# anneouyang/OuterSPACE

Hardware: AMD Instinct MI355X
Metric: spgemm_output_nnz_per_s (higher is better)
Workload: dtype f64

## Files before the change

outerspace_amd/csrc/osp_kernels.h:

```cpp
#pragma once
#include <type_traits>
#include "osp_prims.h"

namespace osp {

template <class T> struct TileCap;
#ifndef OSP_TILE_CAP_F32
#define OSP_TILE_CAP_F32 1792
#endif
template <> struct TileCap<float> { static constexpr int value = OSP_TILE_CAP_F32; };
#ifndef OSP_TILE_CAP_F64
#define OSP_TILE_CAP_F64 1536
#endif
template <> struct TileCap<double> { static constexpr int value = OSP_TILE_CAP_F64; };
constexpr int kMergeThreads = 256;
constexpr int kTileMaxRows = kMergeThreads - 1;
constexpr int kMulThreads = 256;
#ifndef OSP_MUL_PER_WAVE
#define OSP_MUL_PER_WAVE 2048
#endif
constexpr int kMulPerWave = OSP_MUL_PER_WAVE;
constexpr int kMulPerBlock = kMulPerWave * (kMulThreads / kWave);
#ifndef OSP_MUL_BATCH_MAX
#define OSP_MUL_BATCH_MAX 4096
#endif
constexpr int kMulBatchMax = OSP_MUL_BATCH_MAX;
constexpr int kMulBatchAvg = 64;
#ifndef OSP_MUL_TILE_MIN
#define OSP_MUL_TILE_MIN 1024
#endif
#ifndef OSP_MUL_QU_MID
#define OSP_MUL_QU_MID 2
#endif
#ifndef OSP_MUL_QU_HUB
#define OSP_MUL_QU_HUB 1
#endif
constexpr int kMulTileMin = OSP_MUL_TILE_MIN;
constexpr int kMulTileW = 128;

template <class T>
struct __attribute__((packed, aligned(4))) Part {
    uint32_t col;
    T val;
};

template <class T>
struct __attribute__((packed, aligned(4))) PartWords {
    uint32_t w[sizeof(Part<T>) / 4];
    __device__ __forceinline__ uint32_t col() const { return w[0]; }
    __device__ __forceinline__ T val() const {
        if constexpr (sizeof(T) == 8) return (T)__hiloint2double((int)w[2], (int)w[1]);
        else return (T)__uint_as_float(w[1]);
    }
};
template <class T>
__device__ __forceinline__ PartWords<T> load_part_words(const Part<T> *p) { return *reinterpret_cast<const PartWords<T> *>(p); }
template <class T>
__device__ __forceinline__ void store_part_words(Part<T> *p, const PartWords<T> &r) { *reinterpret_cast<PartWords<T> *>(p) = r; }

#ifndef OSP_NT_STAGE
#define OSP_NT_STAGE 1
#endif
template <class T>
__device__ __forceinline__ void stream_store_part(Part<T> *p, uint32_t col, T val) {
#if OSP_NT_STAGE
    if constexpr (sizeof(T) == 8) {
        typedef uint32_t u32x3 __attribute__((ext_vector_type(3), aligned(4)));
        const uint64_t b = (uint64_t)__double_as_longlong((double)val);
        u32x3 v;
        v.x = col; v.y = (uint32_t)b; v.z = (uint32_t)(b >> 32);
        __builtin_nontemporal_store(v, reinterpret_cast<u32x3 *>(p));
    } else {
        typedef uint32_t u32x2 __attribute__((ext_vector_type(2), aligned(4)));
        u32x2 v;
        v.x = col; v.y = __float_as_uint((float)val);
        __builtin_nontemporal_store(v, reinterpret_cast<u32x2 *>(p));
    }
#else
    *p = Part<T>{col, val};
#endif
}

constexpr uint32_t kFlagRange = 1u, kFlagUnsorted = 2u, kFlagDuplicate = 4u, kFlagPtr = 8u;

template <class T, class X>
__device__ __forceinline__ uint64_t upper_bound_dev(const T *a, uint64_t lo, uint64_t hi, X x) {
    while (lo < hi) {
        uint64_t mid = (lo + hi) >> 1;
        if ((X)a[mid] <= x) lo = mid + 1; else hi = mid;
    }
    return lo;
}
template <class T, class X>
__device__ __forceinline__ uint64_t wave_upper_bound(const T *a, uint64_t lo, uint64_t hi, X x) {
    const uint64_t lane = lane_id();
    while (hi - lo > 64) {
        const uint64_t step = (hi - lo) / 64, p = lo + lane * step;
        const int c = __popcll(__ballot((X)a[p] <= x));
        if (c == 0) return lo;
        if (c < 64) hi = lo + (uint64_t)c * step;
        lo = lo + (uint64_t)(c - 1) * step + 1;
    }
    const bool le = lane < hi - lo && (X)a[lo + lane] <= x;
    return lo + (uint64_t)__popcll(__ballot(le));
}
template <class T, class X>
__device__ __forceinline__ uint64_t lower_bound_dev(const T *a, uint64_t lo, uint64_t hi, X x) {
    while (lo < hi) {
        uint64_t mid = (lo + hi) >> 1;
        if ((X)a[mid] < x) lo = mid + 1; else hi = mid;
    }
    return lo;
// ... 439 lines not shown
                            const bool there = q + i < cj;
                            const uint32_t qi = there ? q + i : q;
                            const uint64_t j = jb + qi;
                            av[i] = wave_bcast(av_l, qi);
                            off[i] = there ? wave_bcast(off_l, qi) : kChunkSkip;
                            ok[i] = in && off[i] != kChunkSkip && !(j == j0 && l < la) && !(j == j1 && l >= lb);
                        }
                        bool dir[QU];
                        chunk_dests<T, QU, MODE>(cells, hub, ri, chunk_off, stage, qstage, off, l, l, bc, dst, dir);
#pragma unroll
                        for (int i = 0; i < QU; i++)
                            if (ok[i]) store_dest<T, MODE>(dst[i], off[i], dir[i], bc, av[i] * bv);
                    }
                }
            }
        } else {
            const uint32_t g = kWave / nb;
            const uint32_t jj = (lane * ((65536u + nb - 1) / nb)) >> 16;
            const uint32_t l = lane - jj * nb;
            const bool in = jj < g;
            uint32_t bc = 0; T bv = 0;
            if (in) { bc = b_colidx[bs + l]; bv = b_vals[bs + l]; }
            for (uint64_t jb = j0; jb <= j1; jb += g) {
                const uint64_t j = jb + jj;
                bool ok = in && j <= j1 && !(j == j0 && l < la) && !(j == j1 && l >= lb);
                if (ok) {
                    uint64_t e = as + j;
                    if constexpr (IND) e = elist[e];
                    const uint64_t raw = chunk_off[e - (uint64_t)e0];
                    if (raw != kChunkSkip) {
                        if (DIRECT && (raw & kDirectBit)) store_direct<T, MODE>(cells, hub, qstage, raw, bs, l, bc, a_vals[e] * bv);
                        else stream_store_part(&stage[raw - base + l], bc, a_vals[e] * bv);
                    }
                }
            }
        }
        cur = p0 + b;
    }
    if constexpr (!IND) return;
    }
}

constexpr int kExpandThreads = 256;
constexpr uint32_t kExpandJob = 8192;
struct ExpandJobs {
    const uint32_t *rows; const uint64_t *row_off; const uint8_t *hmode; uint8_t mode_a, mode_b;
    __device__ uint64_t operator()(uint64_t h) const {
        const uint8_t m = hmode[h];
        if (m != mode_a && m != mode_b) return 0ull;
        const uint64_t U = row_off[rows[h] + 1] - row_off[rows[h]];
        return (U + kExpandJob - 1) / kExpandJob;
    }
};
template <class T>
__global__ __launch_bounds__(kExpandThreads) void expand_rows_kernel(
    const uint32_t *__restrict__ rows, uint32_t nlong, const uint64_t *__restrict__ jobbase, const uint64_t *__restrict__ row_off, uint64_t base,
    const uint32_t *__restrict__ rowfirst, const uint64_t *__restrict__ ct_off, const uint32_t *__restrict__ ct_bs, const uint32_t *__restrict__ perm,
    const T *__restrict__ a_vals, const uint32_t *__restrict__ b_colidx, const T *__restrict__ b_vals, Part<T> *__restrict__ stage) {
    const uint64_t job = blockIdx.x;
    if (job >= jobbase[nlong]) return;
    const unsigned lane = lane_id(), w = threadIdx.x >> 6;
    const uint32_t h = (uint32_t)(upper_bound_dev(jobbase, 0, (uint64_t)nlong + 1, job) - 1);
    const uint32_t row = rows[h];
    const uint64_t rbeg = row_off[row], rend = row_off[row + 1];
    constexpr uint32_t per = kExpandJob / (kExpandThreads / kWave);
    const uint64_t p0 = rbeg + (job - jobbase[h]) * kExpandJob + (uint64_t)w * per;
    if (p0 >= rend) return;
    const uint64_t p1 = min(p0 + per, rend);
    const uint32_t c0 = rowfirst[row], c1 = rowfirst[row + 1];
    uint32_t c = (uint32_t)(upper_bound_dev(ct_off, (uint64_t)c0, (uint64_t)c1, p0) - 1);
    constexpr uint32_t kUnroll = 4;
    for (; c < c1; c += kWave) {
        const uint32_t cq = c + lane;
        const bool cv = cq < c1;
        const uint64_t o0 = cv ? ct_off[cq] : ~0ull, o1 = cv ? ct_off[cq + 1] : ~0ull;
        if (wave_bcast(o0, 0u) >= p1) break;
        const uint32_t bsv = cv ? ct_bs[cq] : 0u;
        const T av = cv ? (perm ? a_vals[perm[cq]] : a_vals[cq]) : T(0);
        const uint64_t g0 = max(wave_bcast(o0, 0u), p0);
        const uint32_t nval = min((uint32_t)kWave, c1 - c);
        const uint64_t g1 = min(wave_bcast(o1, nval - 1), p1);
        for (uint64_t ib = g0; ib < g1; ib += kUnroll * kWave) {
            uint32_t bc[kUnroll];
            T bv[kUnroll], cav[kUnroll];
#pragma unroll
            for (uint32_t u = 0; u < kUnroll; u++) {
                const uint64_t i = ib + u * kWave + lane;
                uint32_t lo = 0, hi = kWave;
#pragma unroll
                for (int step = 0; step < 6; step++) {
                    const uint32_t mid = (lo + hi) >> 1;
                    const uint64_t sv = (uint64_t)__shfl((long long)o0, (int)mid);
                    if (sv <= i) lo = mid; else hi = mid;
                }
                const uint64_t cst = (uint64_t)__shfl((long long)o0, (int)lo);
                const uint32_t cbs = (uint32_t)__shfl((int)bsv, (int)lo);
                cav[u] = __shfl(av, (int)lo);
                const uint32_t b = i < g1 ? cbs + (uint32_t)(i - cst) : 0u;
                bc[u] = b_colidx[b];
                bv[u] = b_vals[b];
            }
#pragma unroll
            for (uint32_t u = 0; u < kUnroll; u++) {
                const uint64_t i = ib + u * kWave + lane;
                if (i < g1) stream_store_part(&stage[i - base], bc[u], cav[u] * bv[u]);
            }
        }
    }
}

struct CoarseStartFlag {
    const uint64_t *row_off;
    uint64_t r0, base, slot;
    const uint8_t *force;
    __device__ uint32_t operator()(uint64_t t) const {
        if (t == 0) return 1;
        const uint64_t r = r0 + t;
        if (force && force[t]) return 1;
        return ((row_off[r] - base) / slot != (row_off[r - 1] - base) / slot || (t & 0xffffu) == 0) ? 1u : 0u;
    }
};
__global__ void tile_walk_kernel(const uint32_t *cb_rows, const uint32_t *ncb_p, uint32_t ncb_max, uint64_t r_end, const uint64_t *row_off,
                                 uint64_t cap, uint32_t max_rows, const uint32_t *tile_base, uint32_t *counts,
                                 uint32_t *tile_rows) {
    const uint32_t j = blockIdx.x * blockDim.x + threadIdx.x;
    const uint32_t ncb = *ncb_p;
    if (j >= ncb) {
        if (!tile_rows && j < ncb_max) counts[j] = 0;
        return;
    }
    uint64_t r = cb_rows[j];
    const uint64_t end = (j + 1 < ncb) ? (uint64_t)cb_rows[j + 1] : r_end;
    uint32_t n = 0;
    const uint32_t out = tile_rows ? tile_base[j] : 0u;
    while (r < end) {
        if (tile_rows) tile_rows[out + n] = (uint32_t)r;
        const uint64_t lim = min(end, r + max_rows);
        uint64_t r2 = upper_bound_dev(row_off, r + 1, lim + 1, row_off[r] + cap) - 1;
        if (r2 <= r) r2 = r + 1;
        r = r2;
        n++;
    }
    if (!tile_rows) counts[j] = n;
}
struct HeavyRowFlag {
    const uint64_t *row_off;
    uint64_t r0;
    uint32_t kTileCap;
    __device__ uint32_t operator()(uint64_t t) const {
        const uint64_t r = r0 + t;
        return (row_off[r + 1] - row_off[r]) > (uint64_t)kTileCap ? 1u : 0u;
    }
};
template <class F>
__global__ void compact_flagged_kernel(F f, const uint32_t *scan, uint64_t n, uint64_t r0,
                                       uint32_t *list) {
    uint64_t t = (uint64_t)blockIdx.x * blockDim.x + threadIdx.x;
    if (t < n && f(t)) list[scan[t]] = (uint32_t)(r0 + t);
}

constexpr uint64_t kStatusAgg = 1ull << 62, kStatusPrefix = 2ull << 62, kStatusMask = (1ull << 62) - 1;
// ... 1364 lines not shown
```

outerspace_amd/csrc/osp_pipeline.h:

```cpp
#pragma once

#define OSP_WITH_RA(ctx_, ...)                                               \
    do {                                                                     \
        if ((ctx_)->rank_atomic) { constexpr bool RA = true; __VA_ARGS__; }  \
        else { constexpr bool RA = false; __VA_ARGS__; }                     \
    } while (0)

template <class T> struct Producer {
    virtual ~Producer() {}
    virtual void produce(uint64_t r0, uint64_t r1, bool whole, uint64_t base, uint64_t count,
                         Part<T> *stage, PhaseTimer &tm, const uint32_t *cells = nullptr, Part<T> *qstage = nullptr,
                         const HubArgs *hub = nullptr, bool compact = false, bool has_long = true, bool desc_only = false, bool walk_all = false) = 0;
};

template <class T> struct MergeIO {
    Part<T> *stage;
    const uint64_t *row_off; uint64_t r0, r1, base;
    int64_t *c_rowptr; uint32_t *c_col; T *c_val;
    const uint64_t *out_in; uint64_t *out_out;
    ChunkTable<T> ct{};
    uint32_t *abort_word = nullptr;
    const RunDesc<T> *runs0 = nullptr; const uint32_t *rowfirst0 = nullptr; const uint32_t *b_colidx = nullptr; const T *b_vals = nullptr;
};
template <class T> struct ShortRuns {
// ... 34 lines not shown
    pl.tile_rows = sc.get<uint32_t>((uint64_t)pl.ntiles + 1);
    tile_walk_kernel<<<grid_for(ncb, 128), 128, 0, s>>>(tmp_rows, ncb_p, ncb, r1, row_off, cap, max_rows, cb_cnt, nullptr, pl.tile_rows);
    return pl;
}

struct DirectSrc {
    const uint32_t *rowfirst; const uint64_t *off; const uint32_t *bs; const uint32_t *perm; const uint32_t *b_colidx;
    uint64_t *chunk_off;
    uint64_t direct_max;
    const int64_t *b_rowptr = nullptr;
    uint64_t K = 0, nnz_b = 0;
    Scratch *keep = nullptr;
    mutable HubTables hub{};
    mutable bool hub_refused = false;
    bool gather = false;
    bool expand_rows = false;
    mutable bool chunk_off_ready = true;
    const uint32_t *rows_sorted = nullptr;
    const uint64_t *row_off = nullptr;
    uint64_t rw_cap = 0, nnz = 0;
    void ensure_chunk_off(hipStream_t s) const {
        if (chunk_off_ready) return;
        sym_scatter_offsets_kernel<<<grid_for(nnz, 256), 256, 0, s>>>(perm, off, rows_sorted, row_off, rw_cap, nnz, chunk_off);
        chunk_off_ready = true;
    }
    const void *a_vals = nullptr, *b_vals = nullptr;
    bool av_in_order = false;
    unsigned long long *gstat = nullptr;
};

template <class T> struct PanelPlan {
    Scratch sc;
    TilePlan p0;
    uint32_t max_rows = 0;
    uint64_t *hoff = nullptr, *hscan_tmp = nullptr, *blkbase = nullptr, *hbase = nullptr, *vbase = nullptr, *cellbase = nullptr;
    uint8_t *hbits = nullptr, *hmode = nullptr;
    uint32_t *nstretch = nullptr;
    uint64_t nh = 0, nblocks = 0, nvirt = 0, ncell = 0;
    uint64_t mode_rows[3] = {0, 0, 0}, mode_partials[3] = {0, 0, 0};
    uint32_t *ghist = nullptr, *ghist_tmp = nullptr;
    Part<T> *qstage = nullptr;
    uint64_t *vrow_off = nullptr;
    uint8_t *vfirst = nullptr;
    uint32_t *vcol0 = nullptr, *vcol1 = nullptr;
    uint32_t *cells = nullptr;
    HubArgs hub{};
    GatherArgs<T> ga{};
    uint32_t *vrun_off = nullptr, *vrun_end = nullptr;
    uint32_t *nwritten = nullptr;
    uint64_t *xjobbase = nullptr;
    uint64_t xjobs_bound = 0, xpartials = 0;
    bool expand_ok = false;
    bool may_write = false;
    explicit PanelPlan(Context *c) : sc(c) {}
};

__global__ void mode_totals_kernel(const uint32_t *rows, uint32_t nlong, const uint64_t *row_off, const uint8_t *hmode,
                                   const uint8_t *hsmall, unsigned long long *totals) {
    uint64_t part[3] = {0, 0, 0}, cnt[3] = {0, 0, 0}, nsmall = 0;
    for (uint32_t h = blockIdx.x * blockDim.x + threadIdx.x; h < nlong; h += gridDim.x * blockDim.x) {
        const uint64_t U = row_off[rows[h] + 1] - row_off[rows[h]];
        const uint8_t m = hmode[h];
        nsmall += hsmall[h] ? 1ull : 0ull;
#pragma unroll
        for (int mode = 0; mode < 3; mode++) { part[mode] += m == mode ? U : 0ull; cnt[mode] += m == mode ? 1ull : 0ull; }
    }
    for (uint8_t mode = 0; mode < 3; mode++) {
        const uint64_t p = wave_reduce_sum<uint64_t>(part[mode]), c = wave_reduce_sum<uint64_t>(cnt[mode]);
        if (lane_id() == 0 && c) { atomicAdd(&totals[mode], (unsigned long long)c); atomicAdd(&totals[3 + mode], (unsigned long long)p); }
    }
    nsmall = wave_reduce_sum<uint64_t>(nsmall);
    if (lane_id() == 0 && nsmall) atomicAdd(&totals[6], (unsigned long long)nsmall);
}

template <class T>
static void plan_panel(Context *ctx, Result *res, PhaseTimer &tm, PanelPlan<T> &pl, const uint64_t *row_off, uint64_t r0, uint64_t r1,
                       uint64_t base, uint64_t count, int colbits, const DirectSrc *ds) {
    hipStream_t s = ctx->stream;
    Scratch &sc = pl.sc;
    constexpr uint32_t kCap = (uint32_t)TileCap<T>::value;
    pl.max_rows = (uint32_t)std::min<uint64_t>(kTileMaxRows, colbits >= 32 ? 1ull : (1ull << (32 - colbits)));
    pl.p0 = plan_tiles(ctx, sc, row_off, r0, r1, base, kCap, pl.max_rows, nullptr, count, 0);
    res->info.light_tiles += pl.p0.ntiles - pl.p0.nlong;
    if (!pl.p0.nlong) return;
    const uint32_t nlong = pl.p0.nlong;
    pl.hoff = sc.get<uint64_t>((uint64_t)nlong + 1);
    pl.hscan_tmp = sc.get<uint64_t>(scan_scratch_entries(nlong));
    device_exclusive_scan<HeavyLen, uint64_t>(HeavyLen{pl.p0.long_rows, row_off}, nlong, pl.hoff, pl.hscan_tmp, s);
    pl.hbits = sc.get<uint8_t>(nlong);
    pl.hmode = sc.get<uint8_t>(nlong);
    pl.nstretch = sc.get<uint32_t>(nlong);
    uint32_t *nseg = sc.get<uint32_t>(nlong);
    uint64_t *nhist = sc.get<uint64_t>(nlong), *ncellh = sc.get<uint64_t>(nlong);
    const bool want_gather = ds && ds->gather;
    uint64_t *nrund = want_gather ? sc.get<uint64_t>(nlong) : nullptr, *rdbase = want_gather ? sc.get<uint64_t>((uint64_t)nlong + 1) : nullptr;
    uint64_t nrd = 0;
    pl.blkbase = sc.get<uint64_t>((uint64_t)nlong + 1); pl.hbase = sc.get<uint64_t>((uint64_t)nlong + 1);
    pl.vbase = sc.get<uint64_t>((uint64_t)nlong + 1); pl.cellbase = sc.get<uint64_t>((uint64_t)nlong + 1);
    unsigned long long *totals = (unsigned long long *)sc.get<uint64_t>(7);
    uint8_t *hsmall = sc.get<uint8_t>(nlong);
    SmallLimits small_lim{};
    if (want_gather && !(getenv("OSP_PLAN_SMALL") && atoi(getenv("OSP_PLAN_SMALL")) == 0) &&
        !(getenv("OSP_GATHER_OVER") && atoi(getenv("OSP_GATHER_OVER")) == 0)) {
        small_lim.cells = (uint32_t)std::clamp<long>(getenv("OSP_PLAN_SMALL_CELLS") ? atol(getenv("OSP_PLAN_SMALL_CELLS")) : (long)kSmallCells,
                                                     (long)kSmallCellsMin, (long)kSmallCellsMax);
        small_lim.chunks = (uint32_t)std::clamp<long>(getenv("OSP_PLAN_SMALL_CHUNKS") ? atol(getenv("OSP_PLAN_SMALL_CHUNKS")) : (long)kSmallChunks,
// ... 140 lines not shown
            uint32_t *scan_tmp = tmp.get<uint32_t>(scan_scratch_entries(nb + 1));
            OSP_HIP(hipMemsetAsync(rowstart, 0, nb + 4, s));
            hub_rowstart_kernel<<<grid_for(ds->K, 256), 256, 0, s>>>(ds->b_rowptr, ds->K, rowstart);
            const int sh = colbits - hub_b;
            const HubRunFlag flag{rowstart, ds->b_colidx, sh};
            device_exclusive_scan<HubRunFlag, uint32_t>(flag, nb, sx, scan_tmp, s);
            compact_flagged_kernel<HubRunFlag><<<grid_for(nb, 256), 256, 0, s>>>(flag, sx, nb, 0, runstart);
            hub_runstart_end_kernel<<<1, 1, 0, s>>>(sx + nb, runstart, (uint32_t)nb);
            OSP_HIP(hipMemsetAsync(runblk, 0, (nb + 2) * sizeof(uint16_t), s));
            hub_runblk_kernel<<<std::min(grid_for(nb, 256), 4096u), 256, 0, s>>>(sx + nb, runstart, ds->b_colidx, sh, runblk);
            OSP_HIP(hipStreamSynchronize(s));
            ds->hub.sx = sx; ds->hub.runstart = runstart; ds->hub.runblk = runblk; ds->hub.sh = sh;
        }
        tm.begin(PH_HUB_K, s);
        uint64_t *jobruns = sc.get<uint64_t>(pl.nblocks + 1);
        uint64_t *jobscan_tmp = sc.get<uint64_t>(scan_scratch_entries(pl.nblocks + 1));
        const size_t hub_lds = sizeof(uint32_t) << hub_b;
        hub_plan_kernel<false><<<(unsigned)pl.nblocks, kHubThreads, hub_lds, s>>>(pl.p0.long_rows, nlong, pl.blkbase, pl.hbase, pl.hbits, pl.nstretch, row_off,
                                                                           ds->rowfirst, ds->off, ds->bs, ds->perm, ds->b_colidx, ds->hub, pl.ghist,
                                                                           pl.hoff, jobruns, nullptr, nullptr, nullptr);
        device_exclusive_scan<LoadU32, uint32_t>(LoadU32{pl.ghist}, pl.ncell, pl.ghist, pl.ghist_tmp, s);
        device_exclusive_scan<LoadU64, uint64_t>(LoadU64{jobruns}, pl.nblocks, jobruns, jobscan_tmp, s);
        const uint64_t ncells = d2h(jobruns + pl.nblocks, s);
        if (ncells >= (1ull << 40)) throw Error(OSP_ERR_CAPACITY, "hub rows: too many runs in one panel");
        if (getenv("OSP_VERBOSE"))
            fprintf(stderr, "[osp]   hub rows: %llu rows, %llu products in %llu runs (%.2f records per run), %llu jobs, 2^%d blocks\n",
                    (unsigned long long)pl.mode_rows[kModeStretch], (unsigned long long)pl.mode_partials[kModeStretch], (unsigned long long)ncells,
                    ncells ? (double)pl.mode_partials[kModeStretch] / (double)ncells : 0.0, (unsigned long long)pl.nblocks, hub_b);
        const double min_run = getenv("OSP_HUB_MIN_RUN") ? atof(getenv("OSP_HUB_MIN_RUN")) : 4.0;
        const double run = ncells ? (double)pl.mode_partials[kModeStretch] / (double)ncells : 0.0;
        const bool accept = run >= min_run;
        if (!accept) {
            ds->hub_refused = true;
            tm.end(PH_HUB_K);
        } else {
            uint32_t *hcells = sc.get<uint32_t>(ncells);
            ds->ensure_chunk_off(s);
            hub_plan_kernel<true><<<(unsigned)pl.nblocks, kHubThreads, hub_lds, s>>>(pl.p0.long_rows, nlong, pl.blkbase, pl.hbase, pl.hbits, pl.nstretch, row_off,
                                                                              ds->rowfirst, ds->off, ds->bs, ds->perm, ds->b_colidx, ds->hub, pl.ghist,
                                                                              pl.hoff, nullptr, jobruns, hcells, ds->chunk_off);
            tm.end(PH_HUB_K);
            pl.hub.cells = hcells;
            pl.hub.sx = ds->hub.sx;
            res->info.hub_plan_launches++;
            res->info.hub_cells += ncells;
            res->info.hub_rows += pl.mode_rows[kModeStretch];
            res->info.hub_partials += pl.mode_partials[kModeStretch];
        }
        dbg_sync(s, "plan of the hub rows");
    }
    if (ds && ds->expand_rows) {
        pl.expand_ok = true;
        const bool hubs = pl.hub.cells != nullptr;
        const uint64_t rows_x = pl.mode_rows[kModeSplitRow] + (hubs ? 0 : pl.mode_rows[kModeStretch]);
        pl.xpartials = pl.mode_partials[kModeSplitRow] + (hubs ? 0 : pl.mode_partials[kModeStretch]);
        if (rows_x) {
            pl.xjobbase = sc.get<uint64_t>((uint64_t)nlong + 1);
            device_exclusive_scan<ExpandJobs, uint64_t>(ExpandJobs{pl.p0.long_rows, row_off, pl.hmode, kModeSplitRow, hubs ? kModeSplitRow : kModeStretch},
                                                        nlong, pl.xjobbase, pl.hscan_tmp, s);
            pl.xjobs_bound = pl.xpartials / kExpandJob + rows_x;
        }
    }
}

template <class T>
static void merge_panel(Context *ctx, Result *res, PhaseTimer &tm, const MergeIO<T> &io, int colbits, PanelPlan<T> &pl) {
    hipStream_t s = ctx->stream;
    Scratch &sc = pl.sc;
    constexpr uint32_t kCap = (uint32_t)TileCap<T>::value;
    const uint32_t max_rows = pl.max_rows;
#ifdef OSP_CHECK_DESC
    crumbs_init();
#endif
    const uint64_t r1 = io.r1, base = io.base;
    const TilePlan &p0 = pl.p0;

    MergeLevels<T> lv{};
    lv.stage[0] = io.stage; lv.row_off[0] = io.row_off; lv.base[0] = base; lv.c_rowptr[0] = io.c_rowptr; lv.heavy_nnz[0] = nullptr;
    uint32_t ntot = p0.ntiles;
    TileDesc *desc = nullptr;
    TilePlan p1;
    uint64_t *vbase = pl.vbase;
    int64_t *vptr = nullptr;
    uint64_t *seg_src = nullptr;
    uint32_t *seg_nnz = nullptr;
    Part<T> *qstage = pl.qstage;
    if (p0.nlong) {
        const uint32_t nlong = p0.nlong;
        uint64_t *hoff = pl.hoff, *hscan_tmp = pl.hscan_tmp, *blkbase = pl.blkbase, *hbase = pl.hbase;
        uint8_t *hbits = pl.hbits;
        uint32_t *nstretch = pl.nstretch, *ghist = pl.ghist, *ghist_tmp = pl.ghist_tmp;
        const uint64_t nh = pl.nh, nblocks = pl.nblocks, nvirt = pl.nvirt, ncell = pl.ncell;
        uint64_t *vrow_off = pl.vrow_off;
        uint8_t *vfirst = pl.vfirst;
        if (pl.mode_rows[kModeSplitRow]) {
            tm.begin(PH_SPLIT_K);
            OSP_WITH_RA(ctx, split_row_kernel<T, RA><<<nlong, kSplitRowThreads, 0, s>>>(p0.long_rows, nlong, hbits, pl.hmode, vbase, hoff, io.row_off,
                                                                                     base, colbits, io.stage, qstage, vrow_off));
            tm.end(PH_SPLIT_K);
            res->info.split_launches++;
            res->info.split_partials += pl.mode_partials[kModeSplitRow];
            dbg_sync(s, "split: one-workgroup rows");
        }
        if (nblocks && !pl.hub.cells) {
            split_count_kernel<<<(unsigned)nblocks, kSplitThreads, 0, s>>>(p0.long_rows, nlong, blkbase, hbase, hbits, nstretch, io.row_off,
                                                                         base, colbits, (const char *)io.stage, (uint32_t)sizeof(Part<T>), ghist);
            device_exclusive_scan<LoadU32, uint32_t>(LoadU32{ghist}, ncell, ghist, ghist_tmp, s);
            OSP_WITH_RA(ctx, split_scatter_kernel<T, RA><<<(unsigned)nblocks, kSplitThreads, 0, s>>>(
                                 p0.long_rows, nlong, blkbase, hbase, hbits, nstretch, io.row_off, base, colbits, io.stage, ghist, hoff, qstage));
        }
        dbg_sync(s, "split: stretch rows");
        split_vrows_kernel<<<grid_for(nvirt + 1, 256), 256, 0, s>>>(nlong, vbase, hbase, nstretch, hbits, pl.hmode, colbits, ghist, hoff, nvirt, nh,
                                                                   vrow_off, vfirst, pl.vcol0, pl.vcol1);
        OSP_HIP(hipGetLastError());
        dbg_sync(s, "split: segment offsets");
        p1 = plan_tiles(ctx, sc, vrow_off, 0, nvirt, 0, kCap, max_rows, vfirst, nh, nlong);
        dbg_sync(s, "tiles over the segments");
        vptr = (int64_t *)sc.get<uint64_t>(nvirt + 1);
        lv.stage[1] = qstage; lv.row_off[1] = vrow_off; lv.base[1] = 0; lv.c_rowptr[1] = vptr;
        if (p1.nlong) {
            const uint32_t nseg_long = p1.nlong;
            seg_src = sc.get<uint64_t>(nseg_long);
            seg_nnz = sc.get<uint32_t>(nvirt + 1);
            lv.heavy_nnz[1] = seg_nnz;
            if (pl.ga.runs) {
                uint64_t *xsjob = sc.get<uint64_t>((uint64_t)nseg_long + 1);
                uint64_t *xsjob_tmp = sc.get<uint64_t>(scan_scratch_entries((uint64_t)nseg_long + 1));
                device_exclusive_scan<SegExpandJobs, uint64_t>(SegExpandJobs{p1.long_rows, vrow_off, pl.vrun_off}, nseg_long, xsjob, xsjob_tmp, s);
                const uint64_t job_bound = nh / kExpandJob + nseg_long;
                expand_segments_kernel<T><<<(unsigned)std::min<uint64_t>(job_bound, (uint64_t)ctx->cus * 8), kExpandThreads, 0, s>>>(
                    p1.long_rows, nseg_long, xsjob, vrow_off, pl.vrun_off, pl.vrun_end, pl.ga.runs, pl.ga.b_colidx, pl.ga.b_vals, qstage);
            }
            const uint32_t *rest_list = p1.long_rows;
            uint32_t nrest = nseg_long;
            uint32_t *hscan = sc.get<uint32_t>((uint64_t)nseg_long + 1);
            uint64_t *sscan_tmp = sc.get<uint64_t>(scan_scratch_entries(nseg_long));
            {
                const SegDenseFlag df{p1.long_rows, pl.vcol0, pl.vcol1, getenv("OSP_DENSE_SEG") ? atoi(getenv("OSP_DENSE_SEG")) : 1};
                device_exclusive_scan<SegDenseFlag, uint32_t>(df, nseg_long, hscan, (uint32_t *)sscan_tmp, s);
                const uint32_t ndense = d2h(hscan + nseg_long, s);
                if (ndense) {
                    uint32_t *dense_list = sc.get<uint32_t>(ndense), *others = sc.get<uint32_t>(nseg_long - ndense);
                    seg_split_list_kernel<SegDenseFlag><<<grid_for(nseg_long, 256), 256, 0, s>>>(df, hscan, nseg_long, dense_list, others);
                    if (ctx->dense_atomic[sizeof(T) == 8])
                        dense_segment_kernel<T, true><<<grid_for(ndense, kDenseWaves), kDenseWaves * kWave, 0, s>>>(dense_list, ndense, vrow_off, pl.vcol0, pl.vcol1,
                                                                              qstage, seg_nnz);
                    else
                        dense_segment_kernel<T, false><<<grid_for(ndense, kDenseWaves), kDenseWaves * kWave, 0, s>>>(dense_list, ndense, vrow_off, pl.vcol0, pl.vcol1,
                                                                              qstage, seg_nnz);
                    res->info.dense_segments += ndense;
                    rest_list = others;
                    nrest = nseg_long - ndense;
                }
            }
            dbg_sync(s, "over-long segments: dense accumulation");
            const uint32_t big_cap = getenv("OSP_BIGTILE_CAP") ? std::min<uint32_t>((uint32_t)strtoul(getenv("OSP_BIGTILE_CAP"), nullptr, 10), kBigTileCap)
                                                                : (uint32_t)kBigTileCap;
            uint32_t nhuge = 0, nmid = 0;
            uint32_t *huge_list = nullptr, *mid_list = nullptr;
            if (nrest) {
                const SegHugeFlag hf{rest_list, vrow_off, big_cap};
                device_exclusive_scan<SegHugeFlag, uint32_t>(hf, nrest, hscan, (uint32_t *)sscan_tmp, s);
                nhuge = d2h(hscan + nrest, s);
                nmid = nrest - nhuge;
                huge_list = sc.get<uint32_t>(nhuge);
                mid_list = sc.get<uint32_t>(nmid);
// ... 244 lines not shown
    for (uint32_t p = 0; p < npanels; p++) {
        max_panel = std::max(max_panel, panel_count(p));
        max_rows_panel = std::max(max_rows_panel, bounds[p + 1] - bounds[p]);
    }
    Part<T> *stage = sc.get<Part<T>>(max_panel);
    uint64_t *out_nnz = sc.get<uint64_t>((uint64_t)npanels + 1);
    uint32_t *abort_word = sc.get<uint32_t>(1);
    zero_async(s, {{out_nnz, sizeof(uint64_t)}, {abort_word, sizeof(uint32_t)}});
    auto check_abort = [&](uint32_t flag) {
        if (flag) throw Error(OSP_ERR_HIP, "the merge made no progress for seconds (a tile's predecessors never published their sizes); "
                                           "with several ticket shards that happens when fewer workgroups than shards ever run side by side");
    };
    const bool overlap = npanels > 1 && !(getenv("OSP_PLAN_OVERLAP") && atoi(getenv("OSP_PLAN_OVERLAP")) == 0);
    if (overlap) ctx->need_aux();
    struct AuxScope {
        Context *c; hipStream_t main;
        explicit AuxScope(Context *ctx_) : c(ctx_), main(ctx_->stream) { c->stream = c->aux; }
        ~AuxScope() {
            if (std::uncaught_exceptions()) (void)hipStreamSynchronize(c->aux);
            c->stream = main;
        }
    };
    typedef std::unique_ptr<PanelPlan<T>> PlanPtr;
    auto plan_one = [&](uint32_t p, bool beside) -> PlanPtr {
        const uint64_t r0 = bounds[p], r1 = bounds[p + 1];
        const uint64_t base = panel_base(p), count = panel_count(p);
        PlanPtr pl(new PanelPlan<T>(ctx));
        if (beside) {
            AuxScope scope(ctx);
            OSP_HIP(hipStreamWaitEvent(ctx->stream, ctx->aux_fork, 0));
            tm.begin(PH_MERGE, ctx->stream);
            plan_panel<T>(ctx, res, tm, *pl, d_row_off, r0, r1, base, count, colbits, ds);
            tm.end(PH_MERGE);
            OSP_HIP(hipEventRecord(ctx->aux_join, ctx->stream));
            res->info.plans_overlapped++;
        } else {
            tm.begin(PH_MERGE);
            plan_panel<T>(ctx, res, tm, *pl, d_row_off, r0, r1, base, count, colbits, ds);
            tm.end(PH_MERGE);
        }
        return pl;
    };
    auto multiply_and_plan_next = [&](uint32_t p, PanelPlan<T> &plan, PlanPtr &nxt) {
        const uint64_t r0 = bounds[p], r1 = bounds[p + 1];
        const uint64_t base = panel_base(p), count = panel_count(p);
        if (plan.p0.nlong) plan.qstage = plan.sc.template get<Part<T>>(plan.nh);
        const bool beside = overlap && p + 1 < npanels;
        if (beside) { OSP_HIP(hipEventRecord(ctx->aux_fork, s)); ctx->fork_window = true; ctx->releases_in_fork_window = 0; }
        struct WindowEnd { Context *c; ~WindowEnd() { c->fork_window = false; } } window_end{ctx};
        tm.begin(PH_MUL);
        bool column_major = count != 0 && !(sr && plan.p0.nlong == 0), desc_only = false;
        if (count && plan.xjobbase && plan.xjobs_bound) {
            tm.begin(PH_EXPAND_K);
            expand_rows_kernel<T><<<(unsigned)plan.xjobs_bound, kExpandThreads, 0, s>>>(plan.p0.long_rows, plan.p0.nlong, plan.xjobbase, d_row_off, base, ds->rowfirst,
                                                                                     ds->off, ds->bs, ds->av_in_order ? nullptr : ds->perm, (const T *)ds->a_vals,
                                                                                     ds->b_colidx, (const T *)ds->b_vals, stage);
            tm.end(PH_EXPAND_K);
            res->info.expand_launches++;
            res->info.expand_partials += plan.xpartials;
        }
        if (count && plan.expand_ok) {
            desc_only = true;
            const uint32_t nw = (plan.nwritten && plan.may_write) ? d2h(plan.nwritten, s) : 0u;
            column_major = plan.hub.cells != nullptr || nw != 0 || (plan.mode_rows[kModeDirect] != 0 && plan.ga.runs == nullptr);
        }
        const bool mostly_hub = plan.hub.cells != nullptr && plan.mode_partials[kModeStretch] * 3 >= count;
        if (column_major && ds) ds->ensure_chunk_off(s);
        if (column_major) prod.produce(r0, r1, npanels == 1 && all_rows, base, count, stage, tm, plan.cells, plan.qstage, plan.hub.cells ? &plan.hub : nullptr,
                                       plan.ga.runs != nullptr && !mostly_hub, plan.p0.nlong != 0, desc_only, mostly_hub);
        tm.end(PH_MUL);
        if (beside) {
            ctx->fork_window = false;
            if (ctx->releases_in_fork_window)
                throw Error(OSP_ERR_HIP, "internal: " + std::to_string(ctx->releases_in_fork_window) + " pooled buffers were released between the fork of the "
                                         "second stream and the next panel's plan (the pool is not stream-aware: see Context::fork_window)");
            nxt = plan_one(p + 1, true);
            OSP_HIP(hipStreamWaitEvent(s, ctx->aux_join, 0));
        }
    };
    if (sink) {
        std::vector<uint64_t> h_ub(npanels + 1);
        for (uint32_t p = 0; p <= npanels; p++) h_ub[p] = d2h(ub + (bounds[p] - r_lo), s);
        uint64_t max_out = 1;
        for (uint32_t p = 0; p < npanels; p++) max_out = std::max(max_out, h_ub[p + 1] - h_ub[p]);
        c_col = sc.get<uint32_t>(max_out);
        c_val = sc.get<T>(max_out);
        int64_t *prow = sc.get<int64_t>(max_rows_panel + 1);
        uint64_t *cells = sc.get<uint64_t>(2);
        uint64_t nnz_total = 0;
        PlanPtr cur, nxt;
        for (uint32_t p = 0; p < npanels; p++) {
            const uint64_t r0 = bounds[p], r1 = bounds[p + 1];
            const uint64_t base = panel_base(p);
            if (!cur) cur = plan_one(p, false);
            PanelPlan<T> &plan = *cur;
            multiply_and_plan_next(p, plan, nxt);
            tm.begin(PH_MERGE);
            OSP_HIP(hipMemsetAsync(cells, 0, 2 * sizeof(uint64_t), s));
            MergeIO<T> io{stage, d_row_off, r0, r1, base, prow - r0, c_col, c_val, cells, cells + 1};
            if (ct) io.ct = *ct;
            if (sr) { io.runs0 = sr->runs0; io.rowfirst0 = sr->rowfirst0; io.b_colidx = sr->b_colidx; io.b_vals = sr->b_vals; }
            io.abort_word = abort_word;
            merge_panel<T>(ctx, res, tm, io, colbits, plan);
            tm.end(PH_MERGE);
            uint64_t nnz_p = 0;
            uint32_t aflag = 0;
            { Gather g(s); g.add(&nnz_p, (const uint64_t *)cells + 1); g.add(&aflag, (const uint32_t *)abort_word); g.wait(); }
            check_abort(aflag);
            nnz_total += nnz_p;
            const osp_panel_t pd{r0, r1, nnz_p, prow, c_col, c_val, p, npanels, {0, 0}};
            ctx->ensure_free(2ull << 30);
            if (sink->fn(&pd, sink->user)) throw Error(OSP_ERR_ARG, "panel callback returned non-zero");
// ... 136 lines not shown
```

outerspace_amd/csrc/osp_split.h:

```cpp
#pragma once
#include "osp_kernels.h"

namespace osp {

#ifndef OSP_SPLIT_THREADS
#define OSP_SPLIT_THREADS 256
#endif
constexpr int kSplitThreads = OSP_SPLIT_THREADS;
#ifndef OSP_SPLIT_ROW_THREADS
#define OSP_SPLIT_ROW_THREADS 1024
#endif
#ifndef OSP_SPLIT_ROW_PRE
#define OSP_SPLIT_ROW_PRE 1
#endif
constexpr int kSplitRowThreads = OSP_SPLIT_ROW_THREADS;
#ifndef OSP_SPLIT_ROW_STRETCH
#define OSP_SPLIT_ROW_STRETCH 4096
#endif
constexpr int kSplitRowStretch = OSP_SPLIT_ROW_STRETCH;
#ifndef OSP_SPLIT_STRETCH
#define OSP_SPLIT_STRETCH 4096
#endif
constexpr int kSplitStretch = OSP_SPLIT_STRETCH;
#ifndef OSP_SPLIT_JOB_ROUNDS
// ... 49 lines not shown
    const bool big = U > row_max || b > kSplitRowBits;
    const bool capped = (1ull << b) < want;
    const uint64_t nranges = min(2 * U / cap + 2, (1ull << b) + 1);
    const uint64_t nc = rowfirst != nullptr ? (uint64_t)(rowfirst[rows[h] + 1] - rowfirst[rows[h]]) : 0ull;
    const uint64_t dmax = (capped && direct_max) ? max(direct_max, kDirectDenseMax) : direct_max;
    const bool direct = rowfirst != nullptr && b <= kSplitRowBits && (!big || capped) && U <= dmax && nranges <= (uint64_t)kDirectMaxRanges &&
                        nc * nranges <= kDirectRowCells;
    const uint32_t ns = (big && !direct) ? (uint32_t)((U + kSplitJob - 1) / kSplitJob) : 0u;
    if (ns && hub_b) b = hub_b;
    if (direct && !capped) b = min(b + direct_fine, min(colbits, kDirectFineBits));
    hbits[h] = (uint8_t)b;
    hmode[h] = direct ? kModeDirect : big ? kModeStretch : kModeSplitRow;
    nstretch[h] = ns;
    nseg[h] = direct ? (uint32_t)nranges : 1u << b;
    nhist[h] = (uint64_t)ns << b;
    ncell[h] = direct ? ((1ull << b) + 3) / 4 + nc * nranges : 0ull;
    if (nrund) nrund[h] = direct ? min(nc * nranges, U) : 0ull;
    if (hsmall)
        hsmall[h] = direct && !capped && b <= kSmallFineBits && nc >= 1 && nc <= (uint64_t)sl.chunks && nranges <= (uint64_t)sl.ranges &&
                    nc * nranges <= (uint64_t)sl.cells && U < (1ull << 20);
}
struct HeavyLenIf {
    const uint32_t *rows;
    const uint64_t *row_off;
    const uint8_t *hmode;
    uint8_t mode;
    __device__ uint64_t operator()(uint64_t h) const { return hmode[h] == mode ? row_off[rows[h] + 1] - row_off[rows[h]] : 0ull; }
};
struct LoadU32As64 {
    const uint32_t *p;
    __device__ uint64_t operator()(uint64_t i) const { return p[i]; }
};

struct SplitJob {
    uint32_t h, st, b, nst;
    uint64_t beg, end;
    uint64_t hbase;
};
__device__ __forceinline__ SplitJob split_job(const uint32_t *rows, uint32_t nheavy, const uint64_t *blkbase,
                                              const uint64_t *hbase, const uint8_t *hbits, const uint32_t *nstretch,
                                              const uint64_t *row_off, uint64_t base) {
    SplitJob j;
    j.h = (uint32_t)(upper_bound_dev(blkbase, 0, (uint64_t)nheavy + 1, (uint64_t)blockIdx.x) - 1);
    j.st = (uint32_t)(blockIdx.x - blkbase[j.h]);
    j.b = hbits[j.h];
    j.nst = nstretch[j.h];
    const uint64_t s = row_off[rows[j.h]] - base, e = row_off[rows[j.h] + 1] - base;
    j.beg = s + (uint64_t)j.st * kSplitJob;
    j.end = min(j.beg + (uint64_t)kSplitJob, e);
    j.hbase = hbase[j.h];
    return j;
}

__global__ __launch_bounds__(kSplitThreads) void split_count_kernel(
    const uint32_t *rows, uint32_t nheavy, const uint64_t *blkbase, const uint64_t *hbase, const uint8_t *hbits,
    const uint32_t *nstretch, const uint64_t *row_off, uint64_t base, int colbits, const char *stage, uint32_t rec_bytes,
    uint32_t *ghist) {
    __shared__ uint32_t hist[1 << kSplitMaxBits];
    const SplitJob j = split_job(rows, nheavy, blkbase, hbase, hbits, nstretch, row_off, base);
    const uint32_t nseg = 1u << j.b;
    for (uint32_t d = threadIdx.x; d < nseg; d += kSplitThreads) hist[d] = 0;
    __syncthreads();
    const int sh = colbits - (int)j.b;
    for (uint64_t i = j.beg + threadIdx.x; i < j.end; i += kSplitThreads)
        atomicAdd(&hist[*(const uint32_t *)(stage + i * rec_bytes) >> sh], 1u);
    __syncthreads();
    for (uint32_t d = threadIdx.x; d < nseg; d += kSplitThreads) ghist[j.hbase + (uint64_t)d * j.nst + j.st] = hist[d];
}

__device__ __forceinline__ void wave_match_bits(unsigned digit, int bits, bool valid, unsigned &rank, unsigned &count) {
    const uint64_t vm = __ballot(valid);
    uint32_t plo = (uint32_t)vm, phi = (uint32_t)(vm >> 32);
    for (int b = 0; b < bits; b++) {
        const uint32_t bit = (digit >> b) & 1u;
        const uint64_t m = __ballot(bit != 0);
        const uint32_t sbm = 0u - bit;
        plo &= ~((uint32_t)m ^ sbm);
        phi &= ~((uint32_t)(m >> 32) ^ sbm);
    }
    rank = __builtin_amdgcn_mbcnt_hi(phi, __builtin_amdgcn_mbcnt_lo(plo, 0u));
    count = __popc(plo) + __popc(phi);
}

template <class T, bool RA>
__global__ __launch_bounds__(kSplitThreads) void split_scatter_kernel(
    const uint32_t *rows, uint32_t nheavy, const uint64_t *blkbase, const uint64_t *hbase, const uint8_t *hbits,
    const uint32_t *nstretch, const uint64_t *row_off, uint64_t base, int colbits, const Part<T> *stage,
    const uint32_t *goffs, const uint64_t *hoff, Part<T> *qstage) {
    constexpr int NW = kSplitThreads / kWave;
    constexpr int ITERS = kSplitStretch / kSplitThreads;
    __shared__ alignas(8) uint16_t cnt[NW][1 << kSplitMaxBits];
    __shared__ uint32_t boff[1 << kSplitMaxBits];
    const SplitJob j = split_job(rows, nheavy, blkbase, hbase, hbits, nstretch, row_off, base);
    const uint32_t nseg = 1u << j.b;
    const unsigned lane = lane_id(), w = threadIdx.x >> 6;
    const uint32_t qrow = (uint32_t)hoff[j.h] - goffs[j.hbase];
    for (uint32_t d = threadIdx.x; d < nseg; d += kSplitThreads) {
        boff[d] = qrow + goffs[j.hbase + (uint64_t)d * j.nst + j.st];
#pragma unroll
        for (int ww = 0; ww < NW; ww++) cnt[ww][d] = 0;
    }
    __syncthreads();
    const int sh = colbits - (int)j.b;
    for (uint64_t sb = j.beg; sb < j.end; sb += kSplitStretch) {
        const uint64_t se = min(sb + (uint64_t)kSplitStretch, j.end);
        const uint64_t wbeg = sb + (uint64_t)w * (kSplitStretch / NW);
        uint32_t rk[ITERS];
        PartWords<T> rec[ITERS];
#pragma unroll
        for (int it = 0; it < ITERS; it++) {
            const uint64_t i = wbeg + (uint64_t)it * kWave + lane;
            rec[it] = load_part_words(&stage[i < se ? i : sb]);
        }
#pragma unroll
        for (int it = 0; it < ITERS; it++) {
            const uint64_t i = wbeg + (uint64_t)it * kWave + lane;
            const bool valid = i < se;
            const unsigned d = rec[it].col() >> sh;
            rk[it] = 0;
            if constexpr (RA) {
                const unsigned half = 16u * (d & 1u);
                if (valid) rk[it] = (atomicAdd(&reinterpret_cast<uint32_t *>(cnt[w])[d >> 1], 1u << half) >> half) & 0xffffu;
            } else {
                unsigned r, c;
                wave_match_bits(d, (int)j.b, valid, r, c);
                if (valid) {
                    const uint32_t cur = cnt[w][d];
                    rk[it] = cur + r;
                    if (r == 0) cnt[w][d] = (uint16_t)(cur + c);
                }
            }
        }
        __syncthreads();
        for (uint32_t d = threadIdx.x; d < nseg; d += kSplitThreads) {
            uint32_t total = 0;
#pragma unroll
            for (int ww = 0; ww < NW; ww++) total += cnt[ww][d];
            uint32_t run = 0;
#pragma unroll
            for (int ww = 0; ww < NW; ww++) { const uint32_t c = cnt[ww][d]; cnt[ww][d] = (uint16_t)(run - total); run += c; }
            boff[d] += total;
        }
        __syncthreads();
#pragma unroll
        for (int it = 0; it < ITERS; it++) {
            const uint64_t i = wbeg + (uint64_t)it * kWave + lane;
            if (i < se) {
                const unsigned d = rec[it].col() >> sh;
                const uint32_t dst = boff[d] + (uint32_t)(int32_t)(int16_t)cnt[w][d] + rk[it];
                store_part_words(&qstage[dst], rec[it]);
            }
        }
        __syncthreads();
        for (uint32_t d = threadIdx.x; d < nseg; d += kSplitThreads) {
#pragma unroll
            for (int ww = 0; ww < NW; ww++) cnt[ww][d] = 0;
        }
        __syncthreads();
    }
}

__global__ void split_vrows_kernel(uint32_t nheavy, const uint64_t *vbase, const uint64_t *hbase, const uint32_t *nstretch,
                                   const uint8_t *hbits, const uint8_t *hmode, int colbits,
                                   const uint32_t *goffs, const uint64_t *hoff, uint64_t nvirt, uint64_t nh_total,
                                   uint64_t *vrow_off, uint8_t *vfirst, uint32_t *vcol0, uint32_t *vcol1) {
// ... 936 lines not shown
```

Baseline: 68.53 billion.

## Split stretch rows directly from B instead of staged expanded records

Adds a row-walker abstraction that regenerates partial products straight from A's column offsets and B's rows. The split count and scatter kernels for stretch rows use it instead of reading records staged by the expand kernel, so those rows no longer go through expand. This removes one write and two reads of the staged partial-product buffer for stretch rows. In exchange each partial is recomputed twice, with extra binary-search and shuffle work per element. The path is on by default and can be turned off or moved after the join with an environment variable.

```diff
diff --git a/outerspace_amd/csrc/osp_kernels.h b/outerspace_amd/csrc/osp_kernels.h
--- a/outerspace_amd/csrc/osp_kernels.h
+++ b/outerspace_amd/csrc/osp_kernels.h
@@ -58,6 +58,15 @@
 template <class T>
 __device__ __forceinline__ void store_part_words(Part<T> *p, const PartWords<T> &r) { *reinterpret_cast<PartWords<T> *>(p) = r; }
 
+template <class T>
+__device__ __forceinline__ PartWords<T> part_words(uint32_t col, T val) {
+    PartWords<T> r;
+    r.w[0] = col;
+    if constexpr (sizeof(T) == 8) { r.w[1] = (uint32_t)__double2loint((double)val); r.w[2] = (uint32_t)__double2hiint((double)val); }
+    else r.w[1] = __float_as_uint((float)val);
+    return r;
+}
+
 #ifndef OSP_NT_STAGE
 #define OSP_NT_STAGE 1
 #endif
@@ -603,11 +612,84 @@
         return (U + kExpandJob - 1) / kExpandJob;
     }
 };
+template <class T> struct RowSrc {
+    const uint32_t *rowfirst; const uint64_t *ct_off; const uint32_t *ct_bs; const uint32_t *perm; const T *a_vals;
+    const uint32_t *b_colidx; const T *b_vals;
+};
+constexpr uint32_t kWalkUnroll = 4;
+template <class T, bool VALS> struct RowWalker {
+    const RowSrc<T> &src;
+    const unsigned lane;
+    uint32_t c, c1, nval;
+    uint64_t o0, o1;
+    uint32_t bsv;
+    T av;
+    __device__ __forceinline__ void load_group() {
+        const uint32_t cq = c + lane;
+        const bool cv = cq < c1;
+        o0 = cv ? src.ct_off[cq] : ~0ull;
+        o1 = cv ? src.ct_off[cq + 1] : ~0ull;
+        bsv = cv ? src.ct_bs[cq] : 0u;
+        if constexpr (VALS) av = cv ? (src.perm ? src.a_vals[src.perm[cq]] : src.a_vals[cq]) : T(0);
+        nval = min((uint32_t)kWave, c1 - c);
+    }
+    __device__ __forceinline__ RowWalker(const RowSrc<T> &src_, unsigned lane_, uint32_t c0, uint32_t c1_) : src(src_), lane(lane_), c(c0), c1(c1_) {}
+    __device__ __forceinline__ void seek(uint64_t p) {
+        c = (uint32_t)(wave_upper_bound(src.ct_off, (uint64_t)c, (uint64_t)c1, p) - 1);
+        load_group();
+    }
+    template <int U, class F> __device__ __forceinline__ void block(uint64_t q0, uint64_t q1, F &&f) {
+        uint32_t bc[U];
+        T bv[U], cav[U];
+#pragma unroll
+        for (int u = 0; u < U; u++) { bc[u] = 0u; bv[u] = T(0); cav[u] = T(0); }
+        for (;;) {
+            const uint64_t gend = wave_bcast(o1, nval - 1);
+            const uint64_t gs = max(wave_bcast(o0, 0u), q0), ge = min(gend, q1);
+#pragma unroll
+            for (int u = 0; u < U; u++) {
+                const uint64_t r0 = q0 + (uint64_t)u * kWave;
+                if (!(r0 < ge && r0 + kWave > gs)) continue;
+                const uint64_t i = r0 + lane;
+                uint32_t lo = 0, hi = kWave;
+#pragma unroll
+                for (int step = 0; step < 6; step++) {
+                    const uint32_t mid = (lo + hi) >> 1;
+                    const uint64_t sv = (uint64_t)__shfl((long long)o0, (int)mid);
+                    if (sv <= i) lo = mid; else hi = mid;
+                }
+                const uint64_t cst = (uint64_t)__shfl((long long)o0, (int)lo);
+                const uint32_t cbs = (uint32_t)__shfl((int)bsv, (int)lo);
+                T ca = T(0);
+                if constexpr (VALS) ca = __shfl(av, (int)lo);
+                if (i >= gs && i < ge) {
+                    const uint32_t b = cbs + (uint32_t)(i - cst);
+                    bc[u] = src.b_colidx[b];
+                    if constexpr (VALS) { bv[u] = src.b_vals[b]; cav[u] = ca; }
+                }
+            }
+            if (gend >= q1 || c + kWave >= c1) break;
+            c += kWave;
+            load_group();
+        }
+#pragma unroll
+        for (int u = 0; u < U; u++) {
+            const uint64_t i = q0 + (uint64_t)u * kWave + lane;
+            if (i < q1) f(u, i, bc[u], cav[u] * bv[u]);
+        }
+    }
+};
+template <class T, bool VALS, class F>
+__device__ __forceinline__ void walk_row_slice(const RowSrc<T> &src, unsigned lane, uint32_t c0, uint32_t c1, uint64_t p0, uint64_t p1, F &&f) {
+    RowWalker<T, VALS> wk(src, lane, c0, c1);
+    wk.seek(p0);
+    for (uint64_t q0 = p0; q0 < p1; q0 += kWalkUnroll * kWave)
+        wk.template block<(int)kWalkUnroll>(q0, min(q0 + kWalkUnroll * kWave, p1), [&](int, uint64_t i, uint32_t col, T val) { f(i, col, val); });
+}
 template <class T>
 __global__ __launch_bounds__(kExpandThreads) void expand_rows_kernel(
     const uint32_t *__restrict__ rows, uint32_t nlong, const uint64_t *__restrict__ jobbase, const uint64_t *__restrict__ row_off, uint64_t base,
-    const uint32_t *__restrict__ rowfirst, const uint64_t *__restrict__ ct_off, const uint32_t *__restrict__ ct_bs, const uint32_t *__restrict__ perm,
-    const T *__restrict__ a_vals, const uint32_t *__restrict__ b_colidx, const T *__restrict__ b_vals, Part<T> *__restrict__ stage) {
+    const RowSrc<T> src, Part<T> *__restrict__ stage) {
     const uint64_t job = blockIdx.x;
     if (job >= jobbase[nlong]) return;
     const unsigned lane = lane_id(), w = threadIdx.x >> 6;
@@ -617,47 +699,8 @@
     constexpr uint32_t per = kExpandJob / (kExpandThreads / kWave);
     const uint64_t p0 = rbeg + (job - jobbase[h]) * kExpandJob + (uint64_t)w * per;
     if (p0 >= rend) return;
-    const uint64_t p1 = min(p0 + per, rend);
-    const uint32_t c0 = rowfirst[row], c1 = rowfirst[row + 1];
-    uint32_t c = (uint32_t)(upper_bound_dev(ct_off, (uint64_t)c0, (uint64_t)c1, p0) - 1);
-    constexpr uint32_t kUnroll = 4;
-    for (; c < c1; c += kWave) {
-        const uint32_t cq = c + lane;
-        const bool cv = cq < c1;
-        const uint64_t o0 = cv ? ct_off[cq] : ~0ull, o1 = cv ? ct_off[cq + 1] : ~0ull;
-        if (wave_bcast(o0, 0u) >= p1) break;
-        const uint32_t bsv = cv ? ct_bs[cq] : 0u;
-        const T av = cv ? (perm ? a_vals[perm[cq]] : a_vals[cq]) : T(0);
-        const uint64_t g0 = max(wave_bcast(o0, 0u), p0);
-        const uint32_t nval = min((uint32_t)kWave, c1 - c);
-        const uint64_t g1 = min(wave_bcast(o1, nval - 1), p1);
-        for (uint64_t ib = g0; ib < g1; ib += kUnroll * kWave) {
-            uint32_t bc[kUnroll];
-            T bv[kUnroll], cav[kUnroll];
-#pragma unroll
-            for (uint32_t u = 0; u < kUnroll; u++) {
-                const uint64_t i = ib + u * kWave + lane;
-                uint32_t lo = 0, hi = kWave;
-#pragma unroll
-                for (int step = 0; step < 6; step++) {
-                    const uint32_t mid = (lo + hi) >> 1;
-                    const uint64_t sv = (uint64_t)__shfl((long long)o0, (int)mid);
-                    if (sv <= i) lo = mid; else hi = mid;
-                }
-                const uint64_t cst = (uint64_t)__shfl((long long)o0, (int)lo);
-                const uint32_t cbs = (uint32_t)__shfl((int)bsv, (int)lo);
-                cav[u] = __shfl(av, (int)lo);
-                const uint32_t b = i < g1 ? cbs + (uint32_t)(i - cst) : 0u;
-                bc[u] = b_colidx[b];
-                bv[u] = b_vals[b];
-            }
-#pragma unroll
-            for (uint32_t u = 0; u < kUnroll; u++) {
-                const uint64_t i = ib + u * kWave + lane;
-                if (i < g1) stream_store_part(&stage[i - base], bc[u], cav[u] * bv[u]);
-            }
-        }
-    }
+    walk_row_slice<T, true>(src, lane, src.rowfirst[row], src.rowfirst[row + 1], p0, min(p0 + per, rend),
+                            [&](uint64_t i, uint32_t col, T val) { stream_store_part(&stage[i - base], col, val); });
 }
 
 struct CoarseStartFlag {
diff --git a/outerspace_amd/csrc/osp_pipeline.h b/outerspace_amd/csrc/osp_pipeline.h
--- a/outerspace_amd/csrc/osp_pipeline.h
+++ b/outerspace_amd/csrc/osp_pipeline.h
@@ -110,6 +110,8 @@
     uint64_t xjobs_bound = 0, xpartials = 0;
     bool expand_ok = false;
     bool may_write = false;
+    const DirectSrc *split_from_b = nullptr;
+    bool split_beside = false;
     explicit PanelPlan(Context *c) : sc(c) {}
 };
 
@@ -356,15 +358,40 @@
     if (ds && ds->expand_rows) {
         pl.expand_ok = true;
         const bool hubs = pl.hub.cells != nullptr;
-        const uint64_t rows_x = pl.mode_rows[kModeSplitRow] + (hubs ? 0 : pl.mode_rows[kModeStretch]);
-        pl.xpartials = pl.mode_partials[kModeSplitRow] + (hubs ? 0 : pl.mode_partials[kModeStretch]);
+        const int from_b_env = getenv("OSP_SPLIT_FROM_B") ? atoi(getenv("OSP_SPLIT_FROM_B")) : 1;
+        if (!hubs && pl.nblocks != 0 && from_b_env != 0) pl.split_from_b = ds;
+        pl.split_beside = from_b_env != 2;
+        const bool stretch_x = !hubs && !pl.split_from_b;
+        const uint64_t rows_x = pl.mode_rows[kModeSplitRow] + (stretch_x ? pl.mode_rows[kModeStretch] : 0);
+        pl.xpartials = pl.mode_partials[kModeSplitRow] + (stretch_x ? pl.mode_partials[kModeStretch] : 0);
+        if (getenv("OSP_VERBOSE") && pl.nblocks && !hubs)
+            fprintf(stderr, "[osp]   stretch rows: %llu rows, %llu partial products split %s\n", (unsigned long long)pl.mode_rows[kModeStretch],
+                    (unsigned long long)pl.mode_partials[kModeStretch], pl.split_from_b ? (pl.split_beside ? "from B" : "from B, after the join") : "from staged records");
         if (rows_x) {
             pl.xjobbase = sc.get<uint64_t>((uint64_t)nlong + 1);
-            device_exclusive_scan<ExpandJobs, uint64_t>(ExpandJobs{pl.p0.long_rows, row_off, pl.hmode, kModeSplitRow, hubs ? kModeSplitRow : kModeStretch},
+            device_exclusive_scan<ExpandJobs, uint64_t>(ExpandJobs{pl.p0.long_rows, row_off, pl.hmode, kModeSplitRow, stretch_x ? kModeStretch : kModeSplitRow},
                                                         nlong, pl.xjobbase, pl.hscan_tmp, s);
             pl.xjobs_bound = pl.xpartials / kExpandJob + rows_x;
         }
     }
+}
+
+template <class T>
+static void split_stretch_from_b(Context *ctx, hipStream_t s, const PanelPlan<T> &pl, const uint64_t *row_off, uint64_t base, int colbits) {
+    const DirectSrc *ds = pl.split_from_b;
+    const TilePlan &p0 = pl.p0;
+    const uint32_t nlong = p0.nlong;
+    const uint32_t *perm = ds->av_in_order ? nullptr : ds->perm;
+    const RowSrc<float> cols{ds->rowfirst, ds->off, ds->bs, nullptr, nullptr, ds->b_colidx, nullptr};
+    const RowSrc<T> src{ds->rowfirst, ds->off, ds->bs, perm, (const T *)ds->a_vals, ds->b_colidx, (const T *)ds->b_vals};
+    split_count_kernel<true><<<(unsigned)pl.nblocks, kSplitThreads, 0, s>>>(p0.long_rows, nlong, pl.blkbase, pl.hbase, pl.hbits, pl.nstretch, row_off, base, colbits,
+                                                                          nullptr, 0u, pl.ghist, cols);
+    device_exclusive_scan<LoadU32, uint32_t>(LoadU32{pl.ghist}, pl.ncell, pl.ghist, pl.ghist_tmp, s);
+    OSP_WITH_RA(ctx, split_scatter_kernel<T, RA, true><<<(unsigned)pl.nblocks, kSplitThreads, 0, s>>>(
+                         p0.long_rows, nlong, pl.blkbase, pl.hbase, pl.hbits, pl.nstretch, row_off, base, colbits, nullptr, pl.ghist, pl.hoff, pl.qstage, src));
+    split_vrows_kernel<<<grid_for(pl.nvirt + 1, 256), 256, 0, s>>>(nlong, pl.vbase, pl.hbase, pl.nstretch, pl.hbits, pl.hmode, colbits, pl.ghist, pl.hoff, pl.nvirt,
+                                                                  pl.nh, pl.vrow_off, pl.vfirst, pl.vcol0, pl.vcol1);
+    OSP_HIP(hipGetLastError());
 }
 
 template <class T>
@@ -406,7 +433,8 @@
             res->info.split_partials += pl.mode_partials[kModeSplitRow];
             dbg_sync(s, "split: one-workgroup rows");
         }
-        if (nblocks && !pl.hub.cells) {
+        if (pl.split_from_b && !pl.split_beside) split_stretch_from_b<T>(ctx, s, pl, io.row_off, base, colbits);
+        if (nblocks && !pl.hub.cells && !pl.split_from_b) {
             split_count_kernel<<<(unsigned)nblocks, kSplitThreads, 0, s>>>(p0.long_rows, nlong, blkbase, hbase, hbits, nstretch, io.row_off,
                                                                          base, colbits, (const char *)io.stage, (uint32_t)sizeof(Part<T>), ghist);
             device_exclusive_scan<LoadU32, uint32_t>(LoadU32{ghist}, ncell, ghist, ghist_tmp, s);
@@ -414,8 +442,9 @@
                                  p0.long_rows, nlong, blkbase, hbase, hbits, nstretch, io.row_off, base, colbits, io.stage, ghist, hoff, qstage));
         }
         dbg_sync(s, "split: stretch rows");
-        split_vrows_kernel<<<grid_for(nvirt + 1, 256), 256, 0, s>>>(nlong, vbase, hbase, nstretch, hbits, pl.hmode, colbits, ghist, hoff, nvirt, nh,
-                                                                   vrow_off, vfirst, pl.vcol0, pl.vcol1);
+        if (!pl.split_from_b)
+            split_vrows_kernel<<<grid_for(nvirt + 1, 256), 256, 0, s>>>(nlong, vbase, hbase, nstretch, hbits, pl.hmode, colbits, ghist, hoff, nvirt, nh,
+                                                                       vrow_off, vfirst, pl.vcol0, pl.vcol1);
         OSP_HIP(hipGetLastError());
         dbg_sync(s, "split: segment offsets");
         p1 = plan_tiles(ctx, sc, vrow_off, 0, nvirt, 0, kCap, max_rows, vfirst, nh, nlong);
@@ -766,12 +795,15 @@
         bool column_major = count != 0 && !(sr && plan.p0.nlong == 0), desc_only = false;
         if (count && plan.xjobbase && plan.xjobs_bound) {
             tm.begin(PH_EXPAND_K);
-            expand_rows_kernel<T><<<(unsigned)plan.xjobs_bound, kExpandThreads, 0, s>>>(plan.p0.long_rows, plan.p0.nlong, plan.xjobbase, d_row_off, base, ds->rowfirst,
-                                                                                     ds->off, ds->bs, ds->av_in_order ? nullptr : ds->perm, (const T *)ds->a_vals,
-                                                                                     ds->b_colidx, (const T *)ds->b_vals, stage);
+            const RowSrc<T> src{ds->rowfirst, ds->off, ds->bs, ds->av_in_order ? nullptr : ds->perm, (const T *)ds->a_vals, ds->b_colidx, (const T *)ds->b_vals};
+            expand_rows_kernel<T><<<(unsigned)plan.xjobs_bound, kExpandThreads, 0, s>>>(plan.p0.long_rows, plan.p0.nlong, plan.xjobbase, d_row_off, base, src, stage);
             tm.end(PH_EXPAND_K);
             res->info.expand_launches++;
             res->info.expand_partials += plan.xpartials;
+        }
+        if (count && plan.split_from_b && plan.split_beside) {
+            split_stretch_from_b<T>(ctx, s, plan, d_row_off, base, colbits);
+            dbg_sync(s, "split: stretch rows, from B");
         }
         if (count && plan.expand_ok) {
             desc_only = true;
diff --git a/outerspace_amd/csrc/osp_split.h b/outerspace_amd/csrc/osp_split.h
--- a/outerspace_amd/csrc/osp_split.h
+++ b/outerspace_amd/csrc/osp_split.h
@@ -125,18 +125,28 @@
     return j;
 }
 
+template <bool FROM_B = false>
 __global__ __launch_bounds__(kSplitThreads) void split_count_kernel(
     const uint32_t *rows, uint32_t nheavy, const uint64_t *blkbase, const uint64_t *hbase, const uint8_t *hbits,
     const uint32_t *nstretch, const uint64_t *row_off, uint64_t base, int colbits, const char *stage, uint32_t rec_bytes,
-    uint32_t *ghist) {
+    uint32_t *ghist, const RowSrc<float> src = RowSrc<float>{}) {
     __shared__ uint32_t hist[1 << kSplitMaxBits];
     const SplitJob j = split_job(rows, nheavy, blkbase, hbase, hbits, nstretch, row_off, base);
     const uint32_t nseg = 1u << j.b;
     for (uint32_t d = threadIdx.x; d < nseg; d += kSplitThreads) hist[d] = 0;
     __syncthreads();
     const int sh = colbits - (int)j.b;
-    for (uint64_t i = j.beg + threadIdx.x; i < j.end; i += kSplitThreads)
-        atomicAdd(&hist[*(const uint32_t *)(stage + i * rec_bytes) >> sh], 1u);
+    if constexpr (FROM_B) {
+        constexpr uint32_t per = kSplitJob / (kSplitThreads / kWave);
+        const uint32_t row = rows[j.h];
+        const uint64_t p0 = j.beg + (uint64_t)(threadIdx.x >> 6) * per, p1 = min(p0 + per, j.end);
+        if (p0 < p1)
+            walk_row_slice<float, false>(src, lane_id(), src.rowfirst[row], src.rowfirst[row + 1], base + p0, base + p1,
+                                         [&](uint64_t, uint32_t col, float) { atomicAdd(&hist[col >> sh], 1u); });
+    } else {
+        for (uint64_t i = j.beg + threadIdx.x; i < j.end; i += kSplitThreads)
+            atomicAdd(&hist[*(const uint32_t *)(stage + i * rec_bytes) >> sh], 1u);
+    }
     __syncthreads();
     for (uint32_t d = threadIdx.x; d < nseg; d += kSplitThreads) ghist[j.hbase + (uint64_t)d * j.nst + j.st] = hist[d];
 }
@@ -155,11 +165,11 @@
     count = __popc(plo) + __popc(phi);
 }
 
-template <class T, bool RA>
+template <class T, bool RA, bool FROM_B = false>
 __global__ __launch_bounds__(kSplitThreads) void split_scatter_kernel(
     const uint32_t *rows, uint32_t nheavy, const uint64_t *blkbase, const uint64_t *hbase, const uint8_t *hbits,
     const uint32_t *nstretch, const uint64_t *row_off, uint64_t base, int colbits, const Part<T> *stage,
-    const uint32_t *goffs, const uint64_t *hoff, Part<T> *qstage) {
+    const uint32_t *goffs, const uint64_t *hoff, Part<T> *qstage, const RowSrc<T> src = RowSrc<T>{}) {
     constexpr int NW = kSplitThreads / kWave;
     constexpr int ITERS = kSplitStretch / kSplitThreads;
     __shared__ alignas(8) uint16_t cnt[NW][1 << kSplitMaxBits];
@@ -175,15 +185,34 @@
     }
     __syncthreads();
     const int sh = colbits - (int)j.b;
+    const uint32_t wrow = FROM_B ? rows[j.h] : 0u;
+    RowWalker<T, true> walker(src, lane, FROM_B ? src.rowfirst[wrow] : 0u, FROM_B ? src.rowfirst[wrow + 1] : 0u);
     for (uint64_t sb = j.beg; sb < j.end; sb += kSplitStretch) {
         const uint64_t se = min(sb + (uint64_t)kSplitStretch, j.end);
         const uint64_t wbeg = sb + (uint64_t)w * (kSplitStretch / NW);
         uint32_t rk[ITERS];
         PartWords<T> rec[ITERS];
-#pragma unroll
-        for (int it = 0; it < ITERS; it++) {
-            const uint64_t i = wbeg + (uint64_t)it * kWave + lane;
-            rec[it] = load_part_words(&stage[i < se ? i : sb]);
+        if constexpr (FROM_B) {
+            static_assert(ITERS % (int)kWalkUnroll == 0, "a wave span is whole blocks of the row walker");
+#pragma unroll
+            for (int it = 0; it < ITERS; it++) rec[it] = PartWords<T>{};
+            if (wbeg < se) {
+                const uint64_t wend = min(wbeg + (uint64_t)(kSplitStretch / NW), se);
+                walker.seek(base + wbeg);
+#pragma unroll
+                for (int blk = 0; blk < ITERS / (int)kWalkUnroll; blk++) {
+                    const uint64_t q0 = wbeg + (uint64_t)blk * kWalkUnroll * kWave;
+                    if (q0 < wend)
+                        walker.template block<(int)kWalkUnroll>(base + q0, base + min(q0 + kWalkUnroll * kWave, wend),
+                                                                [&](int u, uint64_t, uint32_t col, T val) { rec[blk * (int)kWalkUnroll + u] = part_words(col, val); });
+                }
+            }
+        } else {
+#pragma unroll
+            for (int it = 0; it < ITERS; it++) {
+                const uint64_t i = wbeg + (uint64_t)it * kWave + lane;
+                rec[it] = load_part_words(&stage[i < se ? i : sb]);
+            }
         }
 #pragma unroll
         for (int it = 0; it < ITERS; it++) {
```

Result: faster. 69.85 billion (median of 6 runs) (+1.9%).
